# myriadrf/LoRa-SDR

Measured on AMD Instinct MI355X. Metric: Msymbols/sec demodulated (dechirp+FFT+argmax), higher is better.
Workload: dtype f32; 1 GPU; batch 4096 channels SF=7 (N=128 FFT) x 256 symbol windows per channel per step, per GPU; sf=7, channels_per_gpu=4096, symbols_per_channel=256, parallelism=channels sharded, 1 rank(s), no data-path collective

## Files before the change

lora_sdr_amd/csrc/lorahip_device.h:

```cpp
#pragma once
#pragma clang fp contract(off)
#include "lorahip_internal.h"

namespace lorahip {

#ifndef LORAHIP_PRIO_ALTERNATE
#define LORAHIP_PRIO_ALTERNATE 18
#endif
#ifndef LORAHIP_PRIO_HOLD
#define LORAHIP_PRIO_HOLD 1
#endif
#ifndef LORAHIP_PRIO_BATCH
#define LORAHIP_PRIO_BATCH 16
#endif
__device__ __forceinline__ int wavefrontSlot()
{
    return int(__builtin_amdgcn_s_getreg((3 << 11) | 4));
}
template <int K>
__device__ __forceinline__ void holdPriority(const bool hold)
{
    if (K > 0 && hold) __builtin_amdgcn_s_setprio(3);
}
template <int WPS, int K>
// ... 170 lines not shown
        for (int j = 0; j < 4; j++) y[j] = fmaLoV(x[i + j], c[i + j], q[j]);
#pragma unroll
        for (int j = 0; j < 4; j++) q[j] = mulHiV(y[j], f);
#pragma unroll
        for (int j = 0; j < 4; j++) x[i + j] = fmaLoV(y[j], f, q[j]);
    }
}
#else
__device__ __forceinline__ void bfly4v(v2f &f0, v2f &f1, v2f &f2, v2f &f3, const v2f t1, const v2f t2, const v2f t3)
{
    const v2f p1 = mulLoV(f1, t1), q1 = mulHiV(f1, t1), p2 = mulLoV(f2, t2), q2 = mulHiV(f2, t2), p3 = mulLoV(f3, t3), q3 = mulHiV(f3, t3);
    const v2f s0 = subAddV(p1, q1), s1 = subAddV(p2, q2), s2 = subAddV(p3, q3);
    bfly4corev(f0, f1, f2, f3, s0, s1, s2);
}
template <int CNT>
__device__ __forceinline__ void dechirpMany(v2f *x, const v2f *c, const v2f f)
{
    static_assert(CNT % 4 == 0, "four values per round");
#pragma unroll
    for (int i = 0; i < CNT; i += 4)
    {
        v2f p[4], q[4], y[4];
#pragma unroll
        for (int j = 0; j < 4; j++) { p[j] = mulLoV(x[i + j], c[i + j]); q[j] = mulHiV(x[i + j], c[i + j]); }
#pragma unroll
        for (int j = 0; j < 4; j++) y[j] = subAddV(p[j], q[j]);
#pragma unroll
        for (int j = 0; j < 4; j++) { p[j] = mulLoV(y[j], f); q[j] = mulHiV(y[j], f); }
#pragma unroll
        for (int j = 0; j < 4; j++) x[i + j] = subAddV(p[j], q[j]);
    }
}
#endif
__device__ __forceinline__ void bfly4unitv(v2f &f0, v2f &f1, v2f &f2, v2f &f3) { bfly4corev(f0, f1, f2, f3, f1, f2, f3); }
__device__ __forceinline__ void bfly2unitv(v2f &f0, v2f &f1)
{
    const v2f v = f1;
    f1 = f0 - v;
    f0 = f0 + v;
}

template <int LOG2N> struct Plan
{
    static constexpr int N = 1 << LOG2N;
    static constexpr int R4 = LOG2N / 2;
    static constexpr bool HAS_R2 = (LOG2N & 1);
    __host__ __device__ static constexpr int pos(int n)
    {
        int p = 0, m = N;
        for (int s = 0; s < R4; s++) { m >>= 2; p += (n & 3) * m; n >>= 2; }
        if (HAS_R2) p += (n & 1);
        return p;
    }
};

__device__ __forceinline__ int fineStep(const int idx, const float d , const int M)
{
    int n = (int)((float)idx - d);
    if (n < 0) n += M;
    else if (n >= M) n -= M;
    return n;
}

__device__ __forceinline__ void argmaxCombine(float &v, int &i, const float ov, const int oi)
{
    const bool take = (ov > v) | ((ov == v) & (oi < i));
    v = take ? ov : v;
    i = take ? oi : i;
}

typedef unsigned v2u __attribute__((ext_vector_type(2)));
template <int T, bool MAX>
__device__ __forceinline__ unsigned groupReduceU(unsigned v)
{
#define LORAHIP_RED_STEP(O) { const unsigned o_ = (O); v = MAX ? (v > o_ ? v : o_) : (v < o_ ? v : o_); }
    if (T >= 2) LORAHIP_RED_STEP(__builtin_amdgcn_mov_dpp(v, 0xB1, 0xf, 0xf, false))
    if (T >= 4) LORAHIP_RED_STEP(__builtin_amdgcn_mov_dpp(v, 0x4E, 0xf, 0xf, false))
    if (T >= 8) LORAHIP_RED_STEP(__builtin_amdgcn_mov_dpp(v, 0x141, 0xf, 0xf, false))
    if (T >= 16) LORAHIP_RED_STEP(__builtin_amdgcn_mov_dpp(v, 0x140, 0xf, 0xf, false))
    if (T >= 32) { const v2u r = __builtin_amdgcn_permlane16_swap(v, v, false, false); v = r.x; LORAHIP_RED_STEP(r.y) }
    if (T >= 64) { const v2u r = __builtin_amdgcn_permlane32_swap(v, v, false, false); v = r.x; LORAHIP_RED_STEP(r.y) }
#undef LORAHIP_RED_STEP
    return v;
}
template <int T>
__device__ __forceinline__ double groupSumF64(double v)
{
#define LORAHIP_SUM_DPP(CTRL) { const unsigned lo_ = __builtin_amdgcn_mov_dpp((unsigned)__double2loint(v), CTRL, 0xf, 0xf, false), \
                                               hi_ = __builtin_amdgcn_mov_dpp((unsigned)__double2hiint(v), CTRL, 0xf, 0xf, false); \
                                v += __hiloint2double((int)hi_, (int)lo_); }
    if (T >= 2) LORAHIP_SUM_DPP(0xB1)
    if (T >= 4) LORAHIP_SUM_DPP(0x4E)
    if (T >= 8) LORAHIP_SUM_DPP(0x141)
    if (T >= 16) LORAHIP_SUM_DPP(0x140)
#undef LORAHIP_SUM_DPP
    if (T >= 32)
    {
        const v2u l = __builtin_amdgcn_permlane16_swap((unsigned)__double2loint(v), (unsigned)__double2loint(v), false, false);
        const v2u h = __builtin_amdgcn_permlane16_swap((unsigned)__double2hiint(v), (unsigned)__double2hiint(v), false, false);
        v = __hiloint2double((int)h.x, (int)l.x) + __hiloint2double((int)h.y, (int)l.y);
    }
    if (T >= 64)
    {
        const v2u l = __builtin_amdgcn_permlane32_swap((unsigned)__double2loint(v), (unsigned)__double2loint(v), false, false);
        const v2u h = __builtin_amdgcn_permlane32_swap((unsigned)__double2hiint(v), (unsigned)__double2hiint(v), false, false);
        v = __hiloint2double((int)h.x, (int)l.x) + __hiloint2double((int)h.y, (int)l.y);
    }
    return v;
}

template <int T>
__device__ __forceinline__ float groupSumF32(float v)
{
#define LORAHIP_SUM_DPP32(CTRL) v += __uint_as_float(__builtin_amdgcn_mov_dpp(__float_as_uint(v), CTRL, 0xf, 0xf, false));
    if (T >= 2) LORAHIP_SUM_DPP32(0xB1)
    if (T >= 4) LORAHIP_SUM_DPP32(0x4E)
    if (T >= 8) LORAHIP_SUM_DPP32(0x141)
// ... 91 lines not shown
    float cv[CH];
    int cj[CH];
    double ct[CH];
#pragma unroll
    for (int c = 0; c < CH; c++) { cv[c] = 0.0f; cj[c] = 0; ct[c] = 0.0; }
#pragma unroll
    for (int k = 0; k < PER; k++)
#pragma unroll
        for (int c = 0; c < CH; c++)
        {
            const int j = c * PER + k;
            const auto b = bin(j);
#ifdef LORAHIP_FMA
            const float mag2 = __builtin_fmaf(b.x, b.x, b.y * b.y);
#else
            const float mag2 = b.x * b.x + b.y * b.y;
#endif
            ct[c] += (double)mag2;
            if (mag2 > cv[c]) { cv[c] = mag2; cj[c] = j; }
        }
#pragma unroll
    for (int w = 1; w < CH; w <<= 1)
#pragma unroll
        for (int c = 0; c + w < CH; c += 2 * w)
        {
            if (cv[c + w] > cv[c]) { cv[c] = cv[c + w]; cj[c] = cj[c + w]; }
            ct[c] += ct[c + w];
        }
    bestV = cv[0];
    tot = ct[0];
    return cj[0];
}

#ifndef LORAHIP_QUICK_SCAN_CHAINS
#define LORAHIP_QUICK_SCAN_CHAINS 1
#endif
template <int CNT, class BIN>
__device__ __forceinline__ int laneScanQuick(BIN bin, float &bestV, float &totF)
{
    constexpr int CH = LORAHIP_QUICK_SCAN_CHAINS, PER = CNT / CH;
    float cv[CH], ct[CH];
    int cj[CH];
#pragma unroll
    for (int c = 0; c < CH; c++) { cv[c] = 0.0f; ct[c] = 0.0f; cj[c] = 0; }
#pragma unroll
    for (int k = 0; k < PER; k++)
#pragma unroll
        for (int c = 0; c < CH; c++)
        {
            const int j = c * PER + k;
            const auto b = bin(j);
#ifdef LORAHIP_FMA
            const float mag2 = __builtin_fmaf(b.x, b.x, b.y * b.y);
#else
            const float mag2 = b.x * b.x + b.y * b.y;
#endif
            ct[c] += mag2;
            if (mag2 > cv[c]) { cv[c] = mag2; cj[c] = j; }
        }
#pragma unroll
    for (int w = 1; w < CH; w <<= 1)
#pragma unroll
        for (int c = 0; c + w < CH; c += 2 * w)
        {
            if (cv[c + w] > cv[c]) { cv[c] = cv[c + w]; cj[c] = cj[c + w]; }
            ct[c] += ct[c + w];
// ... 56 lines not shown
```

lora_sdr_amd/csrc/lorahip_fast.hip:

```cpp
#include "lorahip_fastcore.h"

namespace lorahip {

std::vector<cf32> buildStageTwiddles(const int sf, const std::vector<cf32> &tw)
{
    std::vector<cf32> out;
    for (int b = (sf & 1); b + 2 <= sf; b += 2)
    {
        const int m = 1 << b, fs = 1 << (sf - 2 - b);
        for (int q = 1; q <= 3; q++)
            for (int k = 0; k < m; k++) out.push_back(tw[size_t(k) * fs * q]);
    }
    return out;
}

#ifdef LORAHIP_WG_TIMELINE
__device__ unsigned long long gWaveTimeline[16384][4];
extern "C" int lorahip_debug_wave_timeline(void *out, const size_t bytes)
{
    return hipMemcpyFromSymbol(out, HIP_SYMBOL(gWaveTimeline), bytes < sizeof(gWaveTimeline) ? bytes : sizeof(gWaveTimeline)) == hipSuccess ? 0 : -1;
}
#endif

template <class C, bool DBG, bool UNI>
// ... 8 lines not shown
    typedef FastCore<C> K;
    constexpr int N = C::N, T = C::T, VEC = C::VEC, R = C::R, WPW = C::WPW;
    constexpr int LOG2T = C::LOG2T;
    constexpr int NGL = C::NGL, GL = C::GL;
    constexpr int FS = C::FS, XW = C::XW;
    constexpr int WAVES = 4;

    extern __shared__ __attribute__((aligned(16))) char smemRaw[];
    v2f *sTw = reinterpret_cast<v2f *>(smemRaw);
    v2f *sCh = sTw + C::TWN;
    v2f *sX = sCh + C::CH_ELEMS;
    TailRec *sTail = reinterpret_cast<TailRec *>(sX + WAVES * XW);
    double2 *sFine = reinterpret_cast<double2 *>(sTail + WAVES);
    static_assert(((size_t(C::TWN + C::CH_ELEMS + WAVES * XW) * sizeof(v2f) + WAVES * sizeof(TailRec)) & 15) == 0, "the split tables are read with ds_read_b128");

    const int lane = threadIdx.x & 63;
    const int wave = __builtin_amdgcn_readfirstlane(threadIdx.x >> 6);
    const int wsub = lane >> LOG2T;
    const int t = lane & (T - 1);
    v2f *X = sX + wave * XW;
    TailRec &tr = sTail[wave];

    const v2f *gIq = reinterpret_cast<const v2f *>(a.iq), *gDown = reinterpret_cast<const v2f *>(a.down);
    const v2f *gFine = reinterpret_cast<const v2f *>(a.fine);
    v2f *gDec = reinterpret_cast<v2f *>(a.decOut), *gFft = reinterpret_cast<v2f *>(a.fftOut);

    tr.w[lane] = 0xffffffffu;
    for (int i = threadIdx.x; i < C::TW_LDS; i += blockDim.x) sTw[i] = reinterpret_cast<const v2f *>(ft.twStage)[i];

    typename K::TwR twR;
    K::loadTwR(twR, reinterpret_cast<const v2f *>(ft.twStage), t);
    typename K::TwM twM;
    K::loadTwM(twM, reinterpret_cast<const v2f *>(ft.twStage), t);
    FineLds fl;
    fl.A = nullptr; fl.B = nullptr; fl.split = false;
    if (!UNI) fl = fineLoadLds<C::LOG2N>(sFine, a.fineA, a.fineB, threadIdx.x, blockDim.x);

    const bool perWindowSel = !UNI && a.chirpSel != nullptr;
    const float s0 = (!perWindowSel && a.chirpSelAll == LORAHIP_CHIRP_UP) ? -1.0f : 1.0f;
    v2f ch[C::CH_LDS ? 1 : R][C::CH_LDS ? 1 : VEC];
    if (C::CH_LDS)
    {
        for (int i = threadIdx.x; i < N; i += blockDim.x)
        {
            const v2f c = gDown[i];
            sCh[i] = MAKE2(c.x, s0 * c.y);
        }
    }
    else
    {
#pragma unroll
        for (int r = 0; r < (C::CH_LDS ? 0 : R); r++)
#pragma unroll
            for (int u = 0; u < VEC; u++)
            {
                const v2f c = gDown[VEC * t + u + VEC * T * r];
                ch[r][u] = MAKE2(c.x, s0 * c.y);
            }
    }
    __syncthreads();

    unsigned waveId = blockIdx.x * WAVES + wave, waveCount = gridDim.x * WAVES, setEnd = nSets;
    if (C::XCD_CONTIG && gridDim.x >= 8 && (gridDim.x & 7) == 0)
    {
        const unsigned xcd = blockIdx.x & 7, perXcd = (nSets + 7) / 8;
        waveCount = (gridDim.x >> 3) * WAVES;
// ... 86 lines not shown
            const float sgn = (perWindowSel && sel == LORAHIP_CHIRP_UP) ? -1.0f : 1.0f;
            const v2f *cwf = &cw[0][0];
            const v2f sgn2 = MAKE2(1.0f, sgn);
            const auto chirpOf = [&](const int i) { return cwf[i] * sgn2; };
            const auto chirpRaw = [&](const int i) { return cwf[i]; };
            if (anyMoving)
            {
                if (perWindowSel) dechirpFine<fineSplitLog2H(C::LOG2N), R * VEC>(&x[0][0], chirpOf, &yv[0][0], fl, gFine, dechirp);
                else dechirpFine<fineSplitLog2H(C::LOG2N), R * VEC>(&x[0][0], chirpRaw, &yv[0][0], fl, gFine, dechirp);
            }
            else
            {
#pragma unroll
                for (int r = 0; r < R; r++)
#pragma unroll
                    for (int u = 0; u < VEC; u++)
                    {
                        const v2f y = cmulv(cmulv(x[r][u], chirpOf(r * VEC + u)), fconst);
                        x[r][u] = dechirp ? y : x[r][u];
                    }
            }
            __builtin_amdgcn_fence(__ATOMIC_ACQ_REL, "wavefront");
            __builtin_amdgcn_wave_barrier();
        }
        if (DBG && a.decOut && active)
        {
#pragma unroll
            for (int r = 0; r < R; r++)
#pragma unroll
                for (int u = 0; u < VEC; u++) gDec[(size_t)w * N + VEC * t + u + VEC * T * r] = x[r][u];
        }

        v2f vl[NGL][GL];
        K::fft(x, X, wsub, t, sTw, twR, vl, [&]() { if (C::PREFETCH == 1) issueLoads(set + waveCount < setEnd ? set + waveCount : nSets - 1); }, &twM);

        v2f *F = X + wsub * FS;
        float bestV;
        int bestI;
        double tot;
        K::template scan<true, UNI ? 4 : 1>(vl, F, (DBG && a.fftOut && active) ? gFft + (size_t)w * N : nullptr, t, bestV, bestI, tot);

        v2f leftBin, rightBin;
        K::neighbours(vl, F, bestI, lane, t, leftBin, rightBin);
        if (t == 0 && active)
        {
            const int s = pending + wsub;
            tr.w[s] = w; tr.idx[s] = bestI; tr.val[s] = bestV; tr.tot[s] = tot; tr.l[s] = leftBin; tr.r[s] = rightBin;
        }
        pending += WPW;
        __builtin_amdgcn_fence(__ATOMIC_ACQ_REL, "wavefront");
        __builtin_amdgcn_wave_barrier();
        if (pending == 64)
        {
            const unsigned ww = tr.w[lane];
            if (ww < a.nWindows) detectTail(a, ww, tr.idx[lane], tr.val[lane], tr.tot[lane], tr.l[lane], tr.r[lane]);
            pending = 0;
            __builtin_amdgcn_fence(__ATOMIC_ACQ_REL, "wavefront");
            __builtin_amdgcn_wave_barrier();
            tr.w[lane] = 0xffffffffu;
            __builtin_amdgcn_fence(__ATOMIC_ACQ_REL, "wavefront");
            __builtin_amdgcn_wave_barrier();
        }
    }
    if (pending > 0)
    {
        const unsigned ww = lane < pending ? tr.w[lane] : 0xffffffffu;
        if (ww < a.nWindows) detectTail(a, ww, tr.idx[lane], tr.val[lane], tr.tot[lane], tr.l[lane], tr.r[lane]);
    }
#ifdef LORAHIP_WG_TIMELINE
    if (lane == 0 && blockIdx.x * WAVES + wave < 16384)
    {
        unsigned long long *r = gWaveTimeline[blockIdx.x * WAVES + wave];
        r[0] = tl0; r[1] = wall_clock64();
        r[2] = (unsigned long long)__builtin_amdgcn_s_getreg((31 << 11) | 4) | ((unsigned long long)__builtin_amdgcn_s_getreg((31 << 11) | 20) << 32);
        r[3] = (unsigned long long)tlSets | ((tlLoop - tl0) << 32);
    }
// ... 23 lines not shown
    unsigned grid = (nSets + WAVES - 1) / WAVES;
    if (grid > resident) grid = resident;
    if (grid == 0) return hipSuccess;
    hipLaunchKernelGGL((detectFast<C, DBG, UNI>), dim3(grid), dim3(WAVES * 64), smem, stream, a, ft, nSets);
    return hipGetLastError();
}

template <class C>
static hipError_t launchCfg(const DetectArgs &a, const FastTables &ft, hipStream_t stream)
{
    const bool uni = a.chirpSel == nullptr && a.fineErr == nullptr;
    if (a.decOut || a.fftOut) return launchOne<C, true, false>(a, ft, stream);
    return uni ? launchOne<C, false, true>(a, ft, stream) : launchOne<C, false, false>(a, ft, stream);
}

template <int SF> struct Geo;
template <> struct Geo<6>  { enum { LOG2T = 2, VEC = 4, NPH = 2, PB1 = 2, PB2 = 6, ROT = 2, PAD = 1, S = 0, D = 0 }; };
template <> struct Geo<7>  { enum { LOG2T = 3, VEC = 2, NPH = 2, PB1 = 3, PB2 = 7, ROT = 1, PAD = 1, S = 0, D = 0 }; };
template <> struct Geo<8>  { enum { LOG2T = 4, VEC = 1, NPH = 2, PB1 = 4, PB2 = 8, ROT = 0, PAD = 1, S = 0, D = 0 }; };
template <> struct Geo<9>  { enum { LOG2T = 5, VEC = 2, NPH = 3, PB1 = 3, PB2 = 7, ROT = 2, PAD = 1, S = 1, D = 8 }; };
template <> struct Geo<10> { enum { LOG2T = 6, VEC = 1, NPH = 3, PB1 = 4, PB2 = 8, ROT = 0, PAD = 1, S = 0, D = 0 }; };

enum : unsigned
{
    W2 = 1u << 0, W4 = 1u << 1,
    CH_REG = 1u << 2,
    TW_REG = 1u << 3,
    PF_NONE = 1u << 4, PF_EARLY = 1u << 5,
    NT = 1u << 6,
    NB_SEL = 1u << 7,
    X1_SWAP = 1u << 8,
    TWM_REG = 1u << 9,
    XCD = 1u << 10,
    W1 = 1u << 11
};
template <int SF, unsigned O>
using Fast = FastCfg<SF, Geo<SF>::LOG2T, Geo<SF>::VEC, Geo<SF>::NPH, Geo<SF>::PB1, Geo<SF>::PB2, (O & W2) ? 2 : (O & W4) ? 4 : 3,
                     Geo<SF>::ROT, Geo<SF>::PAD, Geo<SF>::S, Geo<SF>::D, !(O & CH_REG), !(O & TW_REG), (O & PF_NONE) ? 0 : (O & PF_EARLY) ? 2 : 1,
                     (O & NT) != 0, (O & NB_SEL) != 0, (O & X1_SWAP) != 0, (O & TWM_REG) != 0, (O & XCD) != 0>;

template <unsigned O>
using Fast9b = FastCfg<9, 4, 1, 2, 5, 9, (O & W2) ? 2 : (O & W4) ? 4 : 3, 0, 1, 0, 0, !(O & CH_REG), !(O & TW_REG), (O & PF_NONE) ? 0 : (O & PF_EARLY) ? 2 : 1,
                       (O & NT) != 0, (O & NB_SEL) != 0, false, false, false>;

template <unsigned O>
using Fast11q = FastCfg<11, 6, 1, 3, 5, 7, (O & W1) ? 1 : (O & W2) ? 2 : (O & W4) ? 4 : 3, 0, 1, 0, 0, !(O & CH_REG), !(O & TW_REG), (O & PF_NONE) ? 0 : (O & PF_EARLY) ? 2 : 1,
                        (O & NT) != 0, (O & NB_SEL) != 0, false, (O & TWM_REG) != 0, false>;

template <unsigned O>
using Fast10b = FastCfg<10, 4, 1, 2, 6, 10, (O & W1) ? 1 : (O & W2) ? 2 : 3, 0, 1, 0, 0, !(O & CH_REG), !(O & TW_REG), (O & PF_NONE) ? 0 : (O & PF_EARLY) ? 2 : 1,
                        (O & NT) != 0, (O & NB_SEL) != 0, false, false, false>;
template <unsigned O>
using Fast11b = FastCfg<11, 5, 2, 2, 5, 11, (O & W1) ? 1 : (O & W2) ? 2 : 3, 0, 1, 0, 0, !(O & CH_REG), !(O & TW_REG), (O & PF_NONE) ? 0 : (O & PF_EARLY) ? 2 : 1,
                        (O & NT) != 0, (O & NB_SEL) != 0, false, false, false>;
template <unsigned O>
using Fast12b = FastCfg<12, 6, 1, 2, 6, 12, (O & W1) ? 1 : (O & W2) ? 2 : 3, 0, 1, 0, 0, !(O & CH_REG), !(O & TW_REG), (O & PF_NONE) ? 0 : (O & PF_EARLY) ? 2 : 1,
                        (O & NT) != 0, (O & NB_SEL) != 0, false, false, false>;

bool fastAvailable(const int sf) { return sf >= 6 && sf <= 10; }

template <class C>
static bool layoutOk()
{
    std::vector<char> used(size_t(C::XW), 0);
    for (int n = 0; n < C::NL; n++)
        for (int ws = 0; ws < C::WPW; ws++)
            for (int e = 0; e < C::R; e++)
            {
                const int a = C::x0off(n) + ws * C::R + e;
                if (a < 0 || a >= C::XW || used[size_t(a)]) return false;
                used[size_t(a)] = 1;
            }
    return true;
}

bool fastLayoutsOk()
{
    bool ok = layoutOk<Fast<6, 0>>() && layoutOk<Fast<7, 0>>() && layoutOk<Fast<8, 0>>() && layoutOk<Fast<9, 0>>() && layoutOk<Fast9b<0>>() && layoutOk<Fast<10, 0>>();
#ifdef LORAHIP_ALL_VARIANTS
    ok = ok && layoutOk<Fast11q<0>>() && layoutOk<Fast10b<0>>() && layoutOk<Fast11b<0>>() && layoutOk<Fast12b<0>>();
#endif
    return ok;
}

typedef hipError_t (*FastLaunch)(const DetectArgs &, const FastTables &, hipStream_t);

template <class UNI_CFG, class MOVING_CFG, class DBG_CFG>
static hipError_t launchByShape(const DetectArgs &a, const FastTables &ft, hipStream_t stream)
{
    if (a.decOut || a.fftOut) return launchOne<DBG_CFG, true, false>(a, ft, stream);
    const bool uni = a.chirpSel == nullptr && a.fineErr == nullptr;
    return uni ? launchOne<UNI_CFG, false, true>(a, ft, stream) : launchOne<MOVING_CFG, false, false>(a, ft, stream);
}

#ifndef LORAHIP_SF7_MOVING
#define LORAHIP_SF7_MOVING (CH_REG | NT)
#endif
#ifndef LORAHIP_SF10_MOVING
#define LORAHIP_SF10_MOVING (W2 | CH_REG | TW_REG | NT | X1_SWAP | TWM_REG)
#endif
struct FastVariant { int sf, variant; FastLaunch launch; };
#define V(SF, N, OPTS) { SF, N, &launchCfg<Fast<SF, (OPTS)>> }
static const FastVariant kFastVariants[] = {
    { 6, 0, &launchByShape<Fast<6, 0>, Fast<6, 0>, Fast<6, W2>> },
#ifndef LORAHIP_FMA
    { 6, 10, &launchByShape<Fast<6, CH_REG | NT>, Fast<6, CH_REG | NT>, Fast<6, W2 | CH_REG | NT>> },
#endif
    { 7, 0, &launchByShape<Fast<7, CH_REG | NT>, Fast<7, LORAHIP_SF7_MOVING>, Fast<7, W2 | CH_REG | NT>> },
#ifndef LORAHIP_FMA
    { 7, 10, &launchByShape<Fast<7, 0>, Fast<7, 0>, Fast<7, W2>> },
#endif
    { 8, 0, &launchByShape<Fast<8, CH_REG | TW_REG | NT>, Fast<8, W2 | CH_REG | TW_REG | NT | PF_NONE>, Fast<8, W2 | CH_REG | TW_REG | NT | PF_NONE>> },
#ifndef LORAHIP_FMA
    { 8, 10, &launchByShape<Fast<8, 0>, Fast<8, W2>, Fast<8, W2>> },
#endif
    { 9, 0, &launchByShape<Fast9b<W2 | CH_REG | TW_REG | NT | PF_NONE>, Fast<9, W2 | CH_REG | TW_REG | NT | X1_SWAP | TWM_REG>, Fast<9, W2 | CH_REG | TW_REG | NT | X1_SWAP | TWM_REG>> },
#ifndef LORAHIP_FMA
    { 9, 10, &launchByShape<Fast<9, 0>, Fast<9, W2>, Fast<9, W2>> },
#endif
    { 10, 0, &launchByShape<Fast<10, CH_REG | TW_REG | NT | X1_SWAP>, Fast<10, LORAHIP_SF10_MOVING>, Fast<10, W2>> },
#ifndef LORAHIP_FMA
    { 10, 10, &launchByShape<Fast<10, 0>, Fast<10, W2>, Fast<10, W2>> },
#endif
#ifdef LORAHIP_ALL_VARIANTS
    V(6, 7, TW_REG), V(6, 8, NT), V(6, 11, CH_REG | NT), V(6, 12, CH_REG | TW_REG | NT), V(6, 15, CH_REG | TW_REG | NT | PF_NONE),
    V(7, 2, PF_NONE), V(7, 3, W2), V(7, 4, W4 | PF_NONE), V(7, 5, W2 | CH_REG | TW_REG), V(7, 6, PF_EARLY), V(7, 7, TW_REG),
    V(7, 8, NT), V(7, 9, TW_REG | NT), V(7, 11, CH_REG | NT), V(7, 12, W2 | CH_REG | TW_REG | NT),
    V(7, 13, CH_REG | NT | NB_SEL), V(7, 14, CH_REG | NT | XCD), V(7, 15, CH_REG | TW_REG | NT | PF_NONE), V(7, 16, CH_REG | TW_REG | NT | PF_NONE | NB_SEL),
    V(7, 17, W4 | CH_REG | NT | PF_NONE),
    V(8, 6, PF_EARLY), V(8, 7, TW_REG), V(8, 8, NT), V(8, 9, TW_REG | NT), V(8, 11, CH_REG | TW_REG | NT),
    V(8, 13, CH_REG | TW_REG | NT | NB_SEL), V(8, 15, CH_REG | TW_REG | NT | PF_NONE), V(8, 17, W4 | CH_REG | NT | PF_NONE),
    V(9, 6, PF_EARLY), V(9, 7, TW_REG), V(9, 8, NT), V(9, 9, TW_REG | NT), V(9, 11, CH_REG | TW_REG | NT),
    V(9, 12, CH_REG | TW_REG | NT | X1_SWAP), V(9, 13, CH_REG | TW_REG | NT | NB_SEL), V(9, 15, CH_REG | TW_REG | NT | X1_SWAP | TWM_REG | PF_NONE),
    V(9, 16, W2 | CH_REG | TW_REG | NT | X1_SWAP | TWM_REG),
    { 9, 20, &launchCfg<Fast9b<W2 | CH_REG | TW_REG | NT>> }, { 9, 21, &launchCfg<Fast9b<W2 | NT>> }, { 9, 22, &launchCfg<Fast9b<W2 | TW_REG | NT>> },
    { 9, 23, &launchCfg<Fast9b<W2 | CH_REG | NT>> }, { 9, 24, &launchCfg<Fast9b<W2 | CH_REG | TW_REG | NT | PF_NONE>> },
    { 11, 20, &launchCfg<Fast11q<W2 | NT | PF_NONE>> }, { 11, 21, &launchCfg<Fast11q<W2 | TW_REG | NT | PF_NONE>> },
    { 11, 22, &launchCfg<Fast11q<W2 | CH_REG | TW_REG | NT | PF_NONE>> }, { 11, 23, &launchCfg<Fast11q<W2 | NT>> },
    { 11, 24, &launchCfg<Fast11q<W2 | TW_REG | TWM_REG | NT | PF_NONE>> },
    { 10, 25, &launchCfg<Fast10b<W2 | NT | PF_NONE>> }, { 10, 26, &launchCfg<Fast10b<W1 | NT | PF_NONE>> },
    { 11, 25, &launchCfg<Fast11b<W2 | NT | PF_NONE>> }, { 11, 26, &launchCfg<Fast11b<W1 | NT | PF_NONE>> },
// ... 24 lines not shown
```

lora_sdr_amd/csrc/lorahip_fastcore.h:

```cpp
#pragma once
#include "lorahip_fft.h"

namespace lorahip {

template <int LOG2N_, int LOG2T_, int VEC_, int NPH_, int PB1_, int PB2_, int WAVES_PER_SIMD_,
          int X0ROT_, int X0PAD_, int X0S_, int X0D_, bool CH_LDS_, bool TW_ALL_LDS_, int PREFETCH_, bool NT_ = false, bool NB_SELECT_ = false, bool X1_SWAP_ = false, bool TW_MID_REG_ = false, bool XCD_CONTIG_ = false,
          int PB3_ = 0, int X1PAD_ = 8>
struct FastCfg
{
    static constexpr int PREFETCH = PREFETCH_;
    static constexpr bool XCD_CONTIG = XCD_CONTIG_;
    static constexpr bool TW_MID_REG = TW_MID_REG_;
    static constexpr bool X1_SWAP = X1_SWAP_;
    static constexpr bool NB_SELECT = NB_SELECT_;
    static constexpr bool NT = NT_;
    static constexpr bool CH_LDS = CH_LDS_;
    static constexpr bool TW_ALL_LDS = TW_ALL_LDS_;
    static constexpr int LOG2N = LOG2N_, N = 1 << LOG2N_;
    static constexpr int LOG2T = LOG2T_, T = 1 << LOG2T_;
    static constexpr int VEC = VEC_;
    static constexpr int P = N / T;
    static constexpr int R = P / VEC;
    static constexpr int NPH = NPH_;
    static constexpr int WPW = 64 / T;
    static constexpr int WAVES_PER_SIMD = WAVES_PER_SIMD_;
    static constexpr bool HAS_R2 = (LOG2N_ & 1);
    static constexpr int NL = VEC * T;
    static constexpr int LOG2NL = LOG2N_ - PB1_;
    __host__ __device__ static constexpr int bound(const int j)
    {
        return j <= 0 ? 0 : (j >= NPH_ ? LOG2N_ : (j == 1 ? PB1_ : (j == 2 ? PB2_ : PB3_)));
    }
    static_assert(NPH_ >= 2 && NPH_ <= 4, "two to four phases");
    static_assert(NPH_ < 4 || (PB3_ > PB2_ && PB3_ < LOG2N_ && ((PB3_ - PB2_) & 1) == 0), "a fourth phase needs its own boundary, whole radix-4 digits");
    static_assert((1 << PB1_) == R, "phase 0 must cover exactly the bits a lane loads");
    static_assert(((LOG2N_ - PB1_) & 1) == 0, "the low sample digits must be whole radix-4 digits");
    static_assert(T <= 64 && T >= 4, "a window lives inside one wavefront");
    static constexpr int RS0 = WPW * R + X0PAD_;
    __host__ __device__ static constexpr int x0off(const int nlow)
    {
        const int rot = ((nlow >> X0ROT_) | (nlow << (LOG2NL - X0ROT_))) & (NL - 1);
        return rot * RS0 + ((nlow >> X0S_) & 1) * X0D_;
// ... 43 lines not shown
                    const int k = ci + (kl << BL);
                    const int base = twStageOffset(LOG2N, b) + k;
                    twR[g][slot] = twStage[base];
                    twR[g][slot + 1] = twStage[base + (1 << b)];
                    twR[g][slot + 2] = twStage[base + (2 << b)];
                    slot += 3;
                }
        }
    }

    typedef v2f TwM[(C::TW_MID_REG && NPH == 3) ? P / C::G1 : 1][(C::TW_MID_REG && NPH == 3) ? C::MSLOTS : 1];
    static __device__ __forceinline__ void loadTwM(TwM &twM, const v2f *__restrict__ twStage, const int t)
    {
        if (!(C::TW_MID_REG && NPH == 3)) return;
#pragma unroll
        for (int g = 0; g < ((C::TW_MID_REG && NPH == 3) ? P / C::G1 : 0); g++)
        {
            const int klow = (t + T * g) & (R - 1);
            int slot = 0;
#pragma unroll
            for (int b = B1; b < B2; b += 2)
#pragma unroll
                for (int kl = 0; kl < (1 << (b - B1)); kl++)
                {
                    const int base = twStageOffset(LOG2N, b) + klow + (kl << B1);
                    twM[g][slot] = twStage[base];
                    twM[g][slot + 1] = twStage[base + (1 << b)];
                    twM[g][slot + 2] = twStage[base + (2 << b)];
                    slot += 3;
                }
        }
    }

    static __device__ __forceinline__ void load(v2f (&xn)[R][VEC], const v2f *__restrict__ in_, const int t)
    {
#pragma unroll
        for (int r = 0; r < R; r++)
        {
            const v2f *p = in_ + VEC * t + VEC * T * r;
            if (VEC >= 2)
            {
#pragma unroll
                for (int h = 0; h < VEC / 2; h++)
                {
                    const v4f q = C::NT ? __builtin_nontemporal_load(reinterpret_cast<const v4f *>(p) + h) : reinterpret_cast<const v4f *>(p)[h];
                    xn[r][(2 * h) % VEC] = MAKE2(q.x, q.y);
                    xn[r][(2 * h + 1) % VEC] = MAKE2(q.z, q.w);
                }
            }
            else xn[r][0] = C::NT ? __builtin_nontemporal_load(p) : *p;
        }
    }

    static __device__ __forceinline__ void chirpFromLds(v2f (&cw)[R][VEC], const v2f *sCh, const int t)
    {
#pragma unroll
        for (int r = 0; r < R; r++)
        {
            const v2f *p = sCh + VEC * t + VEC * T * r;
            if (VEC >= 2)
            {
#pragma unroll
                for (int h = 0; h < VEC / 2; h++)
                {
                    const v4f q = reinterpret_cast<const v4f *>(p)[h];
                    cw[r][(2 * h) % VEC] = MAKE2(q.x, q.y);
                    cw[r][(2 * h + 1) % VEC] = MAKE2(q.z, q.w);
                }
            }
            else cw[r][0] = *p;
        }
    }

    template <class MID>
    static __device__ __forceinline__ void fft(const v2f (&x)[R][VEC], v2f *X, const int wsub, const int t,
                                               const v2f *sTw, const TwR &twR, v2f (&vl)[NGL][GL], MID mid, const TwM *twMp = nullptr)
    {
        v2f v0[VEC][R];
#pragma unroll
        for (int r = 0; r < R; r++)
#pragma unroll
            for (int u = 0; u < VEC; u++) v0[u][Plan<LOG2N>::pos(VEC * T * r) & (R - 1)] = x[r][u];
        mid();
#pragma unroll
        for (int u = 0; u < VEC; u++) runPhase<LOG2N, 0, B1, false>(v0[u], 0, sTw, nullptr);

        {
            v2f *Xw = X + wsub * R;
#pragma unroll
            for (int u = 0; u < VEC; u++)
            {
                v2f *row = Xw + C::x0off(VEC * t + u);
#pragma unroll
                for (int e = 0; e < R; e++) row[e] = v0[u][e];
            }
        }
        __builtin_amdgcn_fence(__ATOMIC_ACQ_REL, "wavefront");
        __builtin_amdgcn_wave_barrier();

        if (NPH == 2)
        {
            const v2f *Xr = X + wsub * R;
#pragma unroll
            for (int g = 0; g < NGL; g++)
#pragma unroll
                for (int e = 0; e < GL; e++) vl[g][e] = Xr[C::x0off(rev4(e, LOG2N - B1)) + (t + T * g)];
        }
        else
        {
            constexpr int G1 = C::G1;
            constexpr int NG1 = P / G1;
            constexpr int HB = LOG2N - B2;
            v2f v1[NG1][G1];
            const v2f *Xr = X + wsub * R;
#pragma unroll
            for (int g = 0; g < NG1; g++)
            {
                const int ci = t + T * g;
// ... 75 lines not shown
                {
                    const int ci = t + T * g;
                    const v2f *col = X1w + (ci >> B2) * (G2 * C::X1) + (ci & ((1 << B2) - 1));
#pragma unroll
                    for (int e = 0; e < G2; e++) v2[g][e] = col[e * C::X1];
                }
#pragma unroll
                for (int g = 0; g < NG2; g++) runPhase<LOG2N, B2, B3, false>(v2[g], (t + T * g) & ((1 << B2) - 1), sTw, nullptr);
#pragma unroll
                for (int g = 0; g < NG2; g++)
                {
                    const int ci = t + T * g;
                    v2f *col = X1w + (ci >> B2) * (G2 * C::X1) + (ci & ((1 << B2) - 1));
#pragma unroll
                    for (int e = 0; e < G2; e++) col[e * C::X1] = v2[g][e];
                }
                __builtin_amdgcn_fence(__ATOMIC_ACQ_REL, "wavefront");
                __builtin_amdgcn_wave_barrier();
            }
#pragma unroll
            for (int g = 0; g < NGL; g++)
            {
                const int ci = t + T * g;
#pragma unroll
                for (int e = 0; e < GL; e++) vl[g][e] = X1w[((ci >> B2) + (e << (BL - B2))) * C::X1 + (ci & ((1 << B2) - 1))];
            }
            }
        }
        __builtin_amdgcn_fence(__ATOMIC_ACQ_REL, "wavefront");
        __builtin_amdgcn_wave_barrier();
#pragma unroll
        for (int g = 0; g < NGL; g++)
        {
            if (C::TW_ALL_LDS) runPhase<LOG2N, BL, LOG2N, false>(vl[g], t + T * g, sTw, nullptr);
            else runPhase<LOG2N, BL, LOG2N, true>(vl[g], 0, nullptr, twR[C::TW_ALL_LDS ? 0 : g]);
        }
    }

    template <bool STORE_F = true, int CHAINS = 1>
    static __device__ __forceinline__ void scan(const v2f (&vl)[NGL][GL], v2f *F, v2f *fftOut, const int t,
                                                float &bestV, int &bestI, double &tot)
    {
        if (!C::NB_SELECT && STORE_F)
        {
#pragma unroll
            for (int e = 0; e < GL; e++)
#pragma unroll
                for (int g = 0; g < NGL; g++) F[(t + T * g) + (e << BL)] = vl[g][e];
        }
        if (fftOut)
        {
#pragma unroll
            for (int e = 0; e < GL; e++)
#pragma unroll
                for (int g = 0; g < NGL; g++) fftOut[(t + T * g) + (e << BL)] = vl[g][e];
        }
        const int bestJ = laneScan<GL * NGL, CHAINS>([&](const int j) { return vl[j % NGL][j / NGL]; }, bestV, tot);
        bestI = (t + T * (bestJ & (NGL - 1))) + ((bestJ / NGL) << BL);
        if (!(bestV > 0.0f)) bestI = 0;
        groupArgmax<T>(bestV, bestI);
        tot = groupSumF64<T>(tot);
    }

    static constexpr float QUICK_REL_ERR = float(GL * NGL + LOG2T + 2) * 0x1p-24f;
    template <bool STORE_F>
    static __device__ __forceinline__ void scanQuick(const v2f (&vl)[NGL][GL], v2f *F, const int t, float &bestV, int &bestI, float &totF)
    {
        if (!C::NB_SELECT && STORE_F)
        {
#pragma unroll
            for (int e = 0; e < GL; e++)
#pragma unroll
                for (int g = 0; g < NGL; g++) F[(t + T * g) + (e << BL)] = vl[g][e];
        }
        const int bestJ = laneScanQuick<GL * NGL>([&](const int j) { return vl[j % NGL][j / NGL]; }, bestV, totF);
        bestI = (t + T * (bestJ & (NGL - 1))) + ((bestJ / NGL) << BL);
        if (!(bestV > 0.0f)) bestI = 0;
        groupArgmax<T>(bestV, bestI);
        totF = groupSumF32<T>(totF);
    }

    template <bool FROM_REGS = C::NB_SELECT>
    static __device__ __forceinline__ void neighbours(const v2f (&vl)[NGL][GL], const v2f *F, const int bestI, const int lane, const int t,
                                                      v2f &leftBin, v2f &rightBin)
    {
        const int bl = (bestI + N - 1) & (N - 1), br = (bestI + 1) & (N - 1);
        if (FROM_REGS)
        {
            const int cil = bl & ((1 << BL) - 1), cir = br & ((1 << BL) - 1);
            const bool ownL = (cil & (T - 1)) == t;
            const int req = ownL ? ((bl >> BL) * NGL + (cil >> LOG2T)) : ((br >> BL) * NGL + (cir >> LOG2T));
            const v2f mine = selectReg<NGL, GL>(vl, req);
            const int base = lane & ~(T - 1);
            leftBin = MAKE2(__shfl(mine.x, base + (cil & (T - 1)), 64), __shfl(mine.y, base + (cil & (T - 1)), 64));
// ... 21 lines not shown
```

lora_sdr_amd/csrc/lorahip_fft.h:

```cpp
#pragma once
#include "lorahip_device.h"
#include "lorahip_fine.h"

namespace lorahip {

__host__ __device__ constexpr int twStageOffset(const int log2n, const int b)
{
    int off = 0;
    for (int bb = (log2n & 1); bb < b; bb += 2) off += 3 << bb;
    return off;
}

__host__ __device__ constexpr int rev4(int x, const int bits)
{
    int r = 0;
    for (int i = 0; i < bits; i += 2) { r = (r << 2) | (x & 3); x >>= 2; }
    return r;
}

template <int LOG2N, int LO, int HI, bool LAST>
__device__ __forceinline__ void runPhase(v2f (&v)[1 << (HI - LO)], const int klow,
                                         const v2f *__restrict__ TWL, const v2f *twR)
{
    constexpr int G = 1 << (HI - LO);
    constexpr bool R2 = (LO == 0) && (LOG2N & 1);
    if (R2)
    {
#pragma unroll
        for (int i = 0; i < G / 2; i++) bfly2unitv(v[2 * i], v[2 * i + 1]);
    }
    int slot = 0;
#pragma unroll
    for (int b = LO + (R2 ? 1 : 0); b < HI; b += 2)
    {
        const int sh = b - LO;
        const int nkl = 1 << sh;
#pragma unroll
        for (int kl = 0; kl < nkl; kl++)
        {
            v2f t1, t2, t3;
            const bool unit = (LO == 0) && (kl == 0);
            if (!unit)
            {
                if (LAST)
                {
                    t1 = twR[slot]; t2 = twR[slot + 1]; t3 = twR[slot + 2];
                }
                else
                {
                    const int k = klow + (kl << LO);
                    const int base = twStageOffset(LOG2N, b) + k;
                    t1 = TWL[base]; t2 = TWL[base + (1 << b)]; t3 = TWL[base + (2 << b)];
                }
            }
            slot += 3;
#pragma unroll
            for (int hi = 0; hi < (G >> (sh + 2)); hi++)
            {
                const int e0 = kl + (hi << (sh + 2));
                if (unit) bfly4unitv(v[e0], v[e0 + nkl], v[e0 + 2 * nkl], v[e0 + 3 * nkl]);
                else bfly4v(v[e0], v[e0 + nkl], v[e0 + 2 * nkl], v[e0 + 3 * nkl], t1, t2, t3);
            }
        }
    }
}

template <int LOG2N, int LO, int HI>
__host__ __device__ constexpr int lastPhaseSlots()
{
    int s = 0;
    for (int b = LO; b < HI; b += 2) s += 3 << (b - LO);
    return s;
}

template <int NG, int G>
__device__ __forceinline__ v2f selectReg(const v2f (&v)[NG][G], const int idx)
{
    constexpr int CNT = NG * G;
    v2f cur[CNT / 2];
    {
        const bool hi = idx & 1;
#pragma unroll
        for (int i = 0; i < CNT / 2; i++)
        {
            const v2f lo2 = v[(2 * i) % NG][(2 * i) / NG], hi2 = v[(2 * i + 1) % NG][(2 * i + 1) / NG];
            cur[i].x = hi ? hi2.x : lo2.x;
            cur[i].y = hi ? hi2.y : lo2.y;
        }
    }
#pragma unroll
    for (int w = CNT / 4, bit = 1; w >= 1; w >>= 1, bit++)
    {
        const bool hi = (idx >> bit) & 1;
// ... 323 lines not shown
```

Measured before the change: 5467 Msym/s.

## Use packed-key argmax scan and register/scalar twiddles for SF7 uniform path

Adds a key-based argmax for the SF7 uniform kernel. Each bin magnitude's low bits are replaced with its index, so a single integer max reduction across lanes gives the argmax. Neighbour bins are then read from LDS, with an exact fallback scan when key truncation picks the wrong peak. First-phase twiddles are held in SGPRs and fed to packed multiplies through scalar operands, and the first final-phase stage's twiddles are preloaded into registers instead of LDS reads. This trades extra register pressure and an LDS round trip for fewer shuffle/compare steps and fewer LDS twiddle loads.

```diff
diff --git a/lora_sdr_amd/csrc/lorahip_device.h b/lora_sdr_amd/csrc/lorahip_device.h
--- a/lora_sdr_amd/csrc/lorahip_device.h
+++ b/lora_sdr_amd/csrc/lorahip_device.h
@@ -226,6 +226,32 @@
     }
 }
 #endif
+__device__ __forceinline__ v2f mulLoS(const v2f a, const v2f b)
+{
+    v2f p;
+    asm("v_pk_mul_f32 %0, %1, %2 op_sel:[0,0] op_sel_hi:[1,0]" : "=v"(p) : "v"(a), "s"(b));
+    return p;
+}
+__device__ __forceinline__ v2f mulHiS(const v2f a, const v2f b)
+{
+    v2f q;
+    asm("v_pk_mul_f32 %0, %1, %2 op_sel:[1,1] op_sel_hi:[0,1]" : "=v"(q) : "v"(a), "s"(b));
+    return q;
+}
+__device__ __forceinline__ void bfly4s(v2f &f0, v2f &f1, v2f &f2, v2f &f3, const v2f t1, const v2f t2, const v2f t3)
+{
+#ifdef LORAHIP_FMA
+    const v2f q1 = mulHiS(f1, t1), q2 = mulHiS(f2, t2), q3 = mulHiS(f3, t3);
+    v2f s0, s1, s2;
+    asm("v_pk_fma_f32 %0, %1, %2, %3 op_sel:[0,0,0] op_sel_hi:[1,0,1] neg_lo:[0,0,1]" : "=v"(s0) : "v"(f1), "s"(t1), "v"(q1));
+    asm("v_pk_fma_f32 %0, %1, %2, %3 op_sel:[0,0,0] op_sel_hi:[1,0,1] neg_lo:[0,0,1]" : "=v"(s1) : "v"(f2), "s"(t2), "v"(q2));
+    asm("v_pk_fma_f32 %0, %1, %2, %3 op_sel:[0,0,0] op_sel_hi:[1,0,1] neg_lo:[0,0,1]" : "=v"(s2) : "v"(f3), "s"(t3), "v"(q3));
+#else
+    const v2f p1 = mulLoS(f1, t1), q1 = mulHiS(f1, t1), p2 = mulLoS(f2, t2), q2 = mulHiS(f2, t2), p3 = mulLoS(f3, t3), q3 = mulHiS(f3, t3);
+    const v2f s0 = subAddV(p1, q1), s1 = subAddV(p2, q2), s2 = subAddV(p3, q3);
+#endif
+    bfly4corev(f0, f1, f2, f3, s0, s1, s2);
+}
 __device__ __forceinline__ void bfly4unitv(v2f &f0, v2f &f1, v2f &f2, v2f &f3) { bfly4corev(f0, f1, f2, f3, f1, f2, f3); }
 __device__ __forceinline__ void bfly2unitv(v2f &f0, v2f &f1)
 {
@@ -277,6 +303,20 @@
 #undef LORAHIP_RED_STEP
     return v;
 }
+template <int T>
+__device__ __forceinline__ unsigned groupMaxU(unsigned v)
+{
+#define LORAHIP_MAX_DPP(CTRL) { const unsigned o_ = __builtin_amdgcn_update_dpp(0u, v, CTRL, 0xf, 0xf, true); v = v > o_ ? v : o_; }
+    if (T >= 2) LORAHIP_MAX_DPP(0xB1)
+    if (T >= 4) LORAHIP_MAX_DPP(0x4E)
+    if (T >= 8) LORAHIP_MAX_DPP(0x141)
+    if (T >= 16) LORAHIP_MAX_DPP(0x140)
+#undef LORAHIP_MAX_DPP
+    if (T >= 32) { const v2u r = __builtin_amdgcn_permlane16_swap(v, v, false, false); v = r.x > r.y ? r.x : r.y; }
+    if (T >= 64) { const v2u r = __builtin_amdgcn_permlane32_swap(v, v, false, false); v = r.x > r.y ? r.x : r.y; }
+    return v;
+}
+
 template <int T>
 __device__ __forceinline__ double groupSumF64(double v)
 {
@@ -434,6 +474,33 @@
     return cj[0];
 }
 
+__device__ __forceinline__ float mag2f(const v2f b)
+{
+#ifdef LORAHIP_FMA
+    return __builtin_fmaf(b.x, b.x, b.y * b.y);
+#else
+    return b.x * b.x + b.y * b.y;
+#endif
+}
+
+template <int CNT, int CHAINS>
+__device__ __forceinline__ double laneTotalF64(const float (&mag)[CNT])
+{
+    constexpr int CH = CNT >= 2 * CHAINS ? CHAINS : 1, PER = CNT / CH;
+    double ct[CH];
+#pragma unroll
+    for (int c = 0; c < CH; c++) ct[c] = 0.0;
+#pragma unroll
+    for (int k = 0; k < PER; k++)
+#pragma unroll
+        for (int c = 0; c < CH; c++) ct[c] += (double)mag[c * PER + k];
+#pragma unroll
+    for (int w = 1; w < CH; w <<= 1)
+#pragma unroll
+        for (int c = 0; c + w < CH; c += 2 * w) ct[c] += ct[c + w];
+    return ct[0];
+}
+
 #ifndef LORAHIP_QUICK_SCAN_CHAINS
 #define LORAHIP_QUICK_SCAN_CHAINS 1
 #endif
diff --git a/lora_sdr_amd/csrc/lorahip_fast.hip b/lora_sdr_amd/csrc/lorahip_fast.hip
--- a/lora_sdr_amd/csrc/lorahip_fast.hip
+++ b/lora_sdr_amd/csrc/lorahip_fast.hip
@@ -64,6 +64,10 @@
     K::loadTwR(twR, reinterpret_cast<const v2f *>(ft.twStage), t);
     typename K::TwM twM;
     K::loadTwM(twM, reinterpret_cast<const v2f *>(ft.twStage), t);
+    typename K::Tw0 tw0;
+    K::loadTw0(tw0, reinterpret_cast<const v2f *>(ft.twStage));
+    typename K::TwF twF;
+    K::loadTwF(twF, reinterpret_cast<const v2f *>(ft.twStage), t);
     FineLds fl;
     fl.A = nullptr; fl.B = nullptr; fl.split = false;
     if (!UNI) fl = fineLoadLds<C::LOG2N>(sFine, a.fineA, a.fineB, threadIdx.x, blockDim.x);
@@ -216,16 +220,20 @@
         }
 
         v2f vl[NGL][GL];
-        K::fft(x, X, wsub, t, sTw, twR, vl, [&]() { if (C::PREFETCH == 1) issueLoads(set + waveCount < setEnd ? set + waveCount : nSets - 1); }, &twM);
+        K::fft(x, X, wsub, t, sTw, twR, vl, [&]() { if (C::PREFETCH == 1) issueLoads(set + waveCount < setEnd ? set + waveCount : nSets - 1); }, &twM, &tw0, &twF);
 
         v2f *F = X + wsub * FS;
         float bestV;
         int bestI;
         double tot;
-        K::template scan<true, UNI ? 4 : 1>(vl, F, (DBG && a.fftOut && active) ? gFft + (size_t)w * N : nullptr, t, bestV, bestI, tot);
-
         v2f leftBin, rightBin;
-        K::neighbours(vl, F, bestI, lane, t, leftBin, rightBin);
+        if constexpr (C::KEY_SCAN && !DBG) K::template scanKeys<UNI ? 4 : 1>(vl, F, t, bestV, bestI, tot, leftBin, rightBin);
+        else
+        {
+            K::template scan<true, UNI ? 4 : 1>(vl, F, (DBG && a.fftOut && active) ? gFft + (size_t)w * N : nullptr, t, bestV, bestI, tot);
+            K::neighbours(vl, F, bestI, lane, t, leftBin, rightBin);
+        }
+
         if (t == 0 && active)
         {
             const int s = pending + wsub;
@@ -315,12 +323,16 @@
     X1_SWAP = 1u << 8,
     TWM_REG = 1u << 9,
     XCD = 1u << 10,
-    W1 = 1u << 11
+    W1 = 1u << 11,
+    KEYS = 1u << 12,
+    TW0_REG = 1u << 13,
+    TWF_REG = 1u << 14
 };
 template <int SF, unsigned O>
 using Fast = FastCfg<SF, Geo<SF>::LOG2T, Geo<SF>::VEC, Geo<SF>::NPH, Geo<SF>::PB1, Geo<SF>::PB2, (O & W2) ? 2 : (O & W4) ? 4 : 3,
                      Geo<SF>::ROT, Geo<SF>::PAD, Geo<SF>::S, Geo<SF>::D, !(O & CH_REG), !(O & TW_REG), (O & PF_NONE) ? 0 : (O & PF_EARLY) ? 2 : 1,
-                     (O & NT) != 0, (O & NB_SEL) != 0, (O & X1_SWAP) != 0, (O & TWM_REG) != 0, (O & XCD) != 0>;
+                     (O & NT) != 0, (O & NB_SEL) != 0, (O & X1_SWAP) != 0, (O & TWM_REG) != 0, (O & XCD) != 0, 0, 8, (O & KEYS) != 0,
+                     (O & TW0_REG) != 0, (O & TWF_REG) != 0>;
 
 template <unsigned O>
 using Fast9b = FastCfg<9, 4, 1, 2, 5, 9, (O & W2) ? 2 : (O & W4) ? 4 : 3, 0, 1, 0, 0, !(O & CH_REG), !(O & TW_REG), (O & PF_NONE) ? 0 : (O & PF_EARLY) ? 2 : 1,
@@ -376,6 +388,9 @@
     return uni ? launchOne<UNI_CFG, false, true>(a, ft, stream) : launchOne<MOVING_CFG, false, false>(a, ft, stream);
 }
 
+#ifndef LORAHIP_SF7_UNI
+#define LORAHIP_SF7_UNI (CH_REG | NT | KEYS | TW0_REG | TWF_REG)
+#endif
 #ifndef LORAHIP_SF7_MOVING
 #define LORAHIP_SF7_MOVING (CH_REG | NT)
 #endif
@@ -389,7 +404,7 @@
 #ifndef LORAHIP_FMA
     { 6, 10, &launchByShape<Fast<6, CH_REG | NT>, Fast<6, CH_REG | NT>, Fast<6, W2 | CH_REG | NT>> },
 #endif
-    { 7, 0, &launchByShape<Fast<7, CH_REG | NT>, Fast<7, LORAHIP_SF7_MOVING>, Fast<7, W2 | CH_REG | NT>> },
+    { 7, 0, &launchByShape<Fast<7, LORAHIP_SF7_UNI>, Fast<7, LORAHIP_SF7_MOVING>, Fast<7, W2 | CH_REG | NT>> },
 #ifndef LORAHIP_FMA
     { 7, 10, &launchByShape<Fast<7, 0>, Fast<7, 0>, Fast<7, W2>> },
 #endif
diff --git a/lora_sdr_amd/csrc/lorahip_fastcore.h b/lora_sdr_amd/csrc/lorahip_fastcore.h
--- a/lora_sdr_amd/csrc/lorahip_fastcore.h
+++ b/lora_sdr_amd/csrc/lorahip_fastcore.h
@@ -5,9 +5,12 @@
 
 template <int LOG2N_, int LOG2T_, int VEC_, int NPH_, int PB1_, int PB2_, int WAVES_PER_SIMD_,
           int X0ROT_, int X0PAD_, int X0S_, int X0D_, bool CH_LDS_, bool TW_ALL_LDS_, int PREFETCH_, bool NT_ = false, bool NB_SELECT_ = false, bool X1_SWAP_ = false, bool TW_MID_REG_ = false, bool XCD_CONTIG_ = false,
-          int PB3_ = 0, int X1PAD_ = 8>
+          int PB3_ = 0, int X1PAD_ = 8, bool KEY_SCAN_ = false, bool TW0_REG_ = false, bool TWF_REG_ = false>
 struct FastCfg
 {
+    static constexpr bool KEY_SCAN = KEY_SCAN_;
+    static constexpr bool TW0_REG = TW0_REG_;
+    static constexpr bool TWF_REG = TWF_REG_;
     static constexpr int PREFETCH = PREFETCH_;
     static constexpr bool XCD_CONTIG = XCD_CONTIG_;
     static constexpr bool TW_MID_REG = TW_MID_REG_;
@@ -117,6 +120,44 @@
         }
     }
 
+    static constexpr int slots0()
+    {
+        int s = 0;
+        for (int b = (LOG2N & 1); b < B1; b += 2) s += 3 << b;
+        return s;
+    }
+    typedef v2f Tw0[C::TW0_REG ? slots0() : 1];
+    static __device__ __forceinline__ void loadTw0(Tw0 &tw0, const v2f *__restrict__ twStage)
+    {
+#pragma unroll
+        for (int i = 0; i < (C::TW0_REG ? slots0() : 1); i++) tw0[i] = MAKE2(0.0f, 0.0f);
+        if (!C::TW0_REG) return;
+        int slot = 0;
+#pragma unroll
+        for (int b = (LOG2N & 1); b < B1; b += 2)
+#pragma unroll
+            for (int kl = 0; kl < (1 << b); kl++)
+            {
+#pragma unroll
+                for (int q = 0; q < 3; q++)
+                {
+                    const v2f w = twStage[twStageOffset(LOG2N, b) + kl + (q << b)];
+                    tw0[slot + q] = MAKE2(__int_as_float(__builtin_amdgcn_readfirstlane(__float_as_int(w.x))),
+                                          __int_as_float(__builtin_amdgcn_readfirstlane(__float_as_int(w.y))));
+                }
+                slot += 3;
+            }
+    }
+
+    typedef v2f TwF[C::TWF_REG ? NGL : 1][3];
+    static __device__ __forceinline__ void loadTwF(TwF &twF, const v2f *__restrict__ twStage, const int t)
+    {
+#pragma unroll
+        for (int g = 0; g < (C::TWF_REG ? NGL : 0); g++)
+#pragma unroll
+            for (int q = 0; q < 3; q++) twF[g][q] = twStage[twStageOffset(LOG2N, BL) + t + T * g + (q << BL)];
+    }
+
     static __device__ __forceinline__ void load(v2f (&xn)[R][VEC], const v2f *__restrict__ in_, const int t)
     {
 #pragma unroll
@@ -159,7 +200,8 @@
 
     template <class MID>
     static __device__ __forceinline__ void fft(const v2f (&x)[R][VEC], v2f *X, const int wsub, const int t,
-                                               const v2f *sTw, const TwR &twR, v2f (&vl)[NGL][GL], MID mid, const TwM *twMp = nullptr)
+                                               const v2f *sTw, const TwR &twR, v2f (&vl)[NGL][GL], MID mid, const TwM *twMp = nullptr,
+                                               const Tw0 *tw0p = nullptr, const TwF *twFp = nullptr)
     {
         v2f v0[VEC][R];
 #pragma unroll
@@ -168,7 +210,11 @@
             for (int u = 0; u < VEC; u++) v0[u][Plan<LOG2N>::pos(VEC * T * r) & (R - 1)] = x[r][u];
         mid();
 #pragma unroll
-        for (int u = 0; u < VEC; u++) runPhase<LOG2N, 0, B1, false>(v0[u], 0, sTw, nullptr);
+        for (int u = 0; u < VEC; u++)
+        {
+            if (C::TW0_REG) runPhase<LOG2N, 0, B1, true, false, true>(v0[u], 0, nullptr, *tw0p);
+            else runPhase<LOG2N, 0, B1, false>(v0[u], 0, sTw, nullptr);
+        }
 
         {
             v2f *Xw = X + wsub * R;
@@ -310,7 +356,8 @@
 #pragma unroll
         for (int g = 0; g < NGL; g++)
         {
-            if (C::TW_ALL_LDS) runPhase<LOG2N, BL, LOG2N, false>(vl[g], t + T * g, sTw, nullptr);
+            if (C::TW_ALL_LDS && C::TWF_REG) runPhase<LOG2N, BL, LOG2N, false, C::TWF_REG>(vl[g], t + T * g, sTw, (*twFp)[C::TWF_REG ? g : 0]);
+            else if (C::TW_ALL_LDS) runPhase<LOG2N, BL, LOG2N, false>(vl[g], t + T * g, sTw, nullptr);
             else runPhase<LOG2N, BL, LOG2N, true>(vl[g], 0, nullptr, twR[C::TW_ALL_LDS ? 0 : g]);
         }
     }
@@ -338,6 +385,52 @@
         if (!(bestV > 0.0f)) bestI = 0;
         groupArgmax<T>(bestV, bestI);
         tot = groupSumF64<T>(tot);
+    }
+
+    template <int CHAINS>
+    static __device__ __forceinline__ void scanKeys(const v2f (&vl)[NGL][GL], v2f *F, const int t, float &bestV, int &bestI, double &tot,
+                                                    v2f &leftBin, v2f &rightBin)
+    {
+        constexpr int CNT = GL * NGL;
+        static_assert(CNT * T == N && (CNT & (CNT - 1)) == 0 && !C::NB_SELECT, "bin = t + T*j over the whole window, bins staged in F");
+#pragma unroll
+        for (int e = 0; e < GL; e++)
+#pragma unroll
+            for (int g = 0; g < NGL; g++) F[(t + T * g) + (e << BL)] = vl[g][e];
+        float mag[CNT];
+#pragma unroll
+        for (int j = 0; j < CNT; j++) mag[j] = mag2f(vl[j % NGL][j / NGL]);
+        tot = laneTotalF64<CNT, CHAINS>(mag);
+        unsigned km = 0;
+        float vm = 0.0f;
+#pragma unroll
+        for (int j = 0; j < CNT; j++)
+        {
+            const unsigned k = (__float_as_uint(mag[j]) & ~unsigned(CNT - 1)) | unsigned(CNT - 1 - j);
+            km = km > k ? km : k;
+            vm = __builtin_fmaxf(vm, mag[j]);
+        }
+        const unsigned key = (km & ~unsigned(N - 1)) | ((km & unsigned(CNT - 1)) << LOG2T) | unsigned(T - 1 - t);
+        const unsigned kmax = groupMaxU<T>(key);
+        const float V = __uint_as_float(groupMaxU<T>(__float_as_uint(vm)));
+        tot = groupSumF64<T>(tot);
+        bestI = (N - 1) - int(kmax & unsigned(N - 1));
+        bestV = V;
+        __builtin_amdgcn_fence(__ATOMIC_ACQ_REL, "wavefront");
+        __builtin_amdgcn_wave_barrier();
+        const v2f peak = F[bestI];
+        leftBin = F[(bestI + N - 1) & (N - 1)];
+        rightBin = F[(bestI + 1) & (N - 1)];
+        if (__builtin_expect(__any(!(mag2f(peak) == V)), 0))
+        {
+            double totL;
+            const int bestJ = laneScan<CNT, CHAINS>([&](const int j) { return vl[j % NGL][j / NGL]; }, bestV, totL);
+            bestI = (t + T * (bestJ & (NGL - 1))) + ((bestJ / NGL) << BL);
+            if (!(bestV > 0.0f)) bestI = 0;
+            groupArgmax<T>(bestV, bestI);
+            leftBin = F[(bestI + N - 1) & (N - 1)];
+            rightBin = F[(bestI + 1) & (N - 1)];
+        }
     }
 
     static constexpr float QUICK_REL_ERR = float(GL * NGL + LOG2T + 2) * 0x1p-24f;
diff --git a/lora_sdr_amd/csrc/lorahip_fft.h b/lora_sdr_amd/csrc/lorahip_fft.h
--- a/lora_sdr_amd/csrc/lorahip_fft.h
+++ b/lora_sdr_amd/csrc/lorahip_fft.h
@@ -18,10 +18,11 @@
     return r;
 }
 
-template <int LOG2N, int LO, int HI, bool LAST>
+template <int LOG2N, int LO, int HI, bool LAST, bool FIRST_REG = false, bool SCALAR_TW = false>
 __device__ __forceinline__ void runPhase(v2f (&v)[1 << (HI - LO)], const int klow,
                                          const v2f *__restrict__ TWL, const v2f *twR)
 {
+    static_assert(!FIRST_REG || (!LAST && LO > 0), "register twiddles of the first stage: a later phase, the rest from LDS");
     constexpr int G = 1 << (HI - LO);
     constexpr bool R2 = (LO == 0) && (LOG2N & 1);
     if (R2)
@@ -42,7 +43,7 @@
             const bool unit = (LO == 0) && (kl == 0);
             if (!unit)
             {
-                if (LAST)
+                if (LAST || (FIRST_REG && b == LO))
                 {
                     t1 = twR[slot]; t2 = twR[slot + 1]; t3 = twR[slot + 2];
                 }
@@ -59,6 +60,7 @@
             {
                 const int e0 = kl + (hi << (sh + 2));
                 if (unit) bfly4unitv(v[e0], v[e0 + nkl], v[e0 + 2 * nkl], v[e0 + 3 * nkl]);
+                else if (SCALAR_TW) bfly4s(v[e0], v[e0 + nkl], v[e0 + 2 * nkl], v[e0 + 3 * nkl], t1, t2, t3);
                 else bfly4v(v[e0], v[e0 + nkl], v[e0 + 2 * nkl], v[e0 + 3 * nkl], t1, t2, t3);
             }
         }
```

Result: no change. 5502 Msym/s, median of 6 (+0.6%).
